# sbokov/AddingDisparityFiltering

Measured on AMD Instinct MI355X. Metric: filtered Mpixels/s (+ achieved HBM GB/s) on 4K disparity, 1/2/4/8 GPUs vs CPU ref, higher is better.
Workload: dtype f32

## Files before the change

addingdisparityfiltering_amd/csrc/conf_kernels.hip:

```cpp
#include "adf_internal.h"
#include <mutex>
#include <cstdlib>
#include <type_traits>
#include "prep_bodies.h"

#pragma clang fp contract(off)

namespace adf {

namespace {

using namespace tile;
#define ADF_ST(p, v) __builtin_nontemporal_store((v), (p))
constexpr int MAX_RADIUS = 40;

template <class Sum2>
__device__ __forceinline__ float disc_value(int s1, Sum2 sum2, double scale, float roll_off)
{
    const float mean = (float)((double)s1 * scale);
    const float sq = (float)(sum2() * scale);
    const float variance = sq - mean * mean;
    const float v = 1.0f - roll_off * variance;
    return v < 0.0f ? 0.0f : v;
}

__global__ void __launch_bounds__(NT) discontinuity_kernel(DiscArgs a)
{
    extern __shared__ __align__(16) unsigned char smem[];
    const int r = a.radius, k = 2 * r + 1;
    const int IH = TY + 2 * r, IW = TX + 2 * r;
    const int IWP = IW | 1;
    long long* h2 = reinterpret_cast<long long*>(smem);
    int* h1 = reinterpret_cast<int*>(h2 + (size_t)IH * TX);
    int16_t* in = reinterpret_cast<int16_t*>(h1 + (size_t)IH * TX);

    const int tid = threadIdx.x, tx = tid & (TX - 1), ty = tid / TX;
    const int x0 = blockIdx.x * TX, y0 = blockIdx.y * TY;
    const int view = a.only_view >= 0 ? a.only_view : (int)(blockIdx.z & 1);
    const size_t pz = a.only_view >= 0 ? blockIdx.z : (blockIdx.z >> 1);
    const char* base = reinterpret_cast<const char*>(a.disp[view]) + (ptrdiff_t)pz * a.pair_stride[view];
    const int rx = a.rx[view];

    for (int yy = ty; yy < IH; yy += NT / TX) {
        const int gy = reflect101(y0 + yy - r, a.rh);
        const int16_t* row = reinterpret_cast<const int16_t*>(base + (ptrdiff_t)(a.ry + gy) * a.stride[view]) + rx;
        for (int xx = tx; xx < IW; xx += TX)
            in[yy * IWP + xx] = row[reflect101(x0 + xx - r, a.rw)];
    }
    __syncthreads();

    for (int item = tid; item < IH * 8; item += NT) {
        const int yy = item >> 3, xs = (item & 7) * 8;
        const int16_t* p = in + yy * IWP + xs;
        int s1 = 0; long long s2 = 0;
        for (int q = 0; q < k; q++) { const int v = p[q]; s1 += v; s2 += (long long)(v * v); }
        int* o1 = h1 + yy * TX + xs; long long* o2 = h2 + yy * TX + xs;
        o1[0] = s1; o2[0] = s2;
#pragma unroll
        for (int i = 1; i < 8; i++) {
            const int va = p[i + k - 1], vb = p[i - 1];
            s1 += va - vb; s2 += (long long)(va * va - vb * vb);
            o1[i] = s1; o2[i] = s2;
        }
    }
    __syncthreads();

    {
        const int ys = ty * 8;
        const double scale = 1.0 / ((double)k * (double)k);
        int s1 = 0; long long s2 = 0;
        for (int q = 0; q < k; q++) { s1 += h1[(ys + q) * TX + tx]; s2 += h2[(ys + q) * TX + tx]; }
        float* dst = a.dst[view] + pz * a.frame;
        const int gx = x0 + tx;
#pragma unroll
        for (int i = 0; i < 8; i++) {
            if (i > 0) {
                s1 += h1[(ys + i + k - 1) * TX + tx] - h1[(ys + i - 1) * TX + tx];
                s2 += h2[(ys + i + k - 1) * TX + tx] - h2[(ys + i - 1) * TX + tx];
            }
            const int gy = y0 + ys + i;
            if (gy < a.rh && gx < a.rw) {
                dst[(size_t)(a.ry + gy) * a.W + rx + gx] = disc_value(s1, [=] { return (double)s2; }, scale, a.roll_off);
            }
        }
    }
}

constexpr int CONF_GROUP = 8;
constexpr int LRC_GROUP = 4;
#define DC_ROWS ((rows_total + (int)gridDim.y - 1) / (int)gridDim.y)

inline int row_blocks(int rows, int blocks_xz)
{
    int rpb = 128;
    while (rpb > 16 && ((rows + rpb - 1) / rpb) * blocks_xz < 2048) rpb >>= 1;
    return (rows + rpb - 1) / rpb;
}

__device__ __forceinline__ void lds_barrier()
{
    asm volatile("s_waitcnt lgkmcnt(0)\n\ts_barrier" ::: "memory");
}

struct WinSum {
    int s1, lo, hi;
    __device__ __forceinline__ void clear() { s1 = 0; lo = 0; hi = 0; }
    __device__ __forceinline__ void tap(const int2 v) { s1 += v.x; lo += v.y & 0xffff; hi += (int)((unsigned)v.y >> 16); }
    __device__ __forceinline__ void add(const WinSum& o) { s1 += o.s1; lo += o.lo; hi += o.hi; }
    __device__ __forceinline__ void sub(const WinSum& o) { s1 -= o.s1; lo -= o.lo; hi -= o.hi; }
    __device__ __forceinline__ double sum2() const { return (double)hi * 65536.0 + (double)lo; }
    __device__ static __forceinline__ int2 stage(int d) { return make_int2(d, __mul24(d, d)); }
};

template <int RT>
__global__ void __launch_bounds__(NT) discontinuity_col_kernel(DiscArgs a)
{
    constexpr int K = 2 * RT + 1;
    constexpr int OUTW = NT - 2 * RT;
    __shared__ int2 rowbuf[2][NT];
    const int tid = threadIdx.x;
    const int rows_total = a.rh;
    const int view = a.only_view >= 0 ? a.only_view : (int)(blockIdx.z & 1);
    const size_t pz = a.only_view >= 0 ? blockIdx.z : (blockIdx.z >> 1);
    const int x_out0 = blockIdx.x * OUTW, y_out0 = blockIdx.y * DC_ROWS;
    const char* base = reinterpret_cast<const char*>(a.disp[view]) + (ptrdiff_t)pz * a.pair_stride[view];
    const int rx = a.rx[view];
    const int gx_in = reflect101(x_out0 - RT + tid, a.rw);
    const int gx_out = x_out0 + tid - RT;
    const bool writer = tid >= RT && tid < NT - RT && gx_out < a.rw;
    float* dst = a.dst[view] + pz * a.frame + (size_t)a.ry * a.W + rx + gx_out;
    const int nrows = min(DC_ROWS, a.rh - y_out0) + 2 * RT;
    const double scale = 1.0 / ((double)K * (double)K);

    auto load = [&](int n) -> int {
        const int gy = reflect101(y_out0 - RT + n, a.rh);
        return reinterpret_cast<const int16_t*>(base + (ptrdiff_t)(a.ry + gy) * a.stride[view])[rx + gx_in];
    };

    constexpr int U = K * ((CONF_GROUP + K - 1) / K);
    WinSum ring[K], S;
    S.clear();
    int nxt[U];
#pragma unroll
    for (int s = 0; s < U; s++) nxt[s] = (s < nrows) ? load(s) : 0;
    for (int n0 = 0; n0 < nrows; n0 += U) {
        int cur[U];
#pragma unroll
        for (int s = 0; s < U; s++) { cur[s] = nxt[s]; asm volatile("" : "+v"(cur[s])); }
#pragma unroll
        for (int s = 0; s < U; s++) nxt[s] = (n0 + U + s < nrows) ? load(n0 + U + s) : 0;
#pragma unroll
        for (int s = 0; s < U; s++) {
            const int n = n0 + s;
            const int slot = s % K;
            if (n < nrows) {
                rowbuf[n & 1][tid] = WinSum::stage(cur[s]);
                lds_barrier();
                WinSum hsum;
                hsum.clear();
                if (tid >= RT && tid < NT - RT) {
#pragma unroll
                    for (int d = -RT; d <= RT; d++) hsum.tap(rowbuf[n & 1][tid + d]);
                }
                if (n >= K) S.sub(ring[slot]);
                ring[slot] = hsum;
                S.add(hsum);
                if (n >= 2 * RT && writer) {
                    const int oy = y_out0 + n - 2 * RT;
                    ADF_ST(&dst[(size_t)oy * a.W], disc_value(S.s1, [&] { return S.sum2(); }, scale, a.roll_off));
                }
            }
        }
    }
}

template <int RT, bool WRITE_U>
__global__ void __launch_bounds__(NT) conf_left_kernel(ConfLeftArgs a)
{
    constexpr int K = 2 * RT + 1;
    constexpr int OUTW = NT - 2 * RT;
    constexpr int U = K * ((LRC_GROUP + K - 1) / K);
    constexpr int CR = RT > 0 ? RT : 1;
    __shared__ int2 rowbuf[2][NT];
    const Geom& g = a.g;
    const int tid = threadIdx.x;
    const int rows_total = g.rh;
    const size_t pz = blockIdx.z;
    const int x_out0 = blockIdx.x * OUTW, y_out0 = blockIdx.y * DC_ROWS;
    const char* baseL = reinterpret_cast<const char*>(a.dL) + (ptrdiff_t)pz * a.psL;
    const char* baseR = reinterpret_cast<const char*>(a.dR) + (ptrdiff_t)pz * a.psR;
    const float* cR = a.cR + pz * g.frame;
    float* conf = a.conf + pz * g.cframe + g.cx0;
    const int gx_in = reflect101(x_out0 - RT + tid, g.rw);
    const int gx_out = x_out0 + tid - RT;
    const bool writer = tid >= RT && tid < NT - RT && gx_out < g.rw;
    const int j_abs = g.rx + gx_out;
    const int rows_out = min(DC_ROWS, g.rh - y_out0);
    const int nrows = rows_out + 2 * RT;
    const double scale = 1.0 / ((double)K * (double)K);
    const int right_end = a.rrx + g.rw;

    auto load = [&](int n) -> int {
        const int gy = reflect101(y_out0 - RT + n, g.rh);
        return reinterpret_cast<const int16_t*>(baseL + (ptrdiff_t)(g.ry + gy) * a.sL)[g.rx + gx_in];
    };

    WinSum ring[K], S;
    S.clear();
    int nxt[U], cur[U];
    int gd[U]; float gc[U];
    int cd[CR], cdr[CR]; float ccr[CR];
#pragma unroll
    for (int k = 0; k < CR; k++) { cd[k] = 0; cdr[k] = 0; ccr[k] = 0.0f; }
#pragma unroll
    for (int s = 0; s < U; s++) nxt[s] = (s < nrows) ? load(s) : 0;
    for (int n0 = 0; n0 < nrows; n0 += U) {
#pragma unroll
        for (int s = 0; s < U; s++) { cur[s] = nxt[s]; asm volatile("" : "+v"(cur[s])); }
#pragma unroll
        for (int s = 0; s < U; s++) {
            const int n = n0 + s;
            gd[s] = 0; gc[s] = 0.0f;
            if (writer && n >= RT && n < nrows - RT) {
                const int ridx = j_abs - (cur[s] >> 4);
                if (ridx >= a.rrx && ridx < right_end) {
                    const int i_abs = g.ry + y_out0 + n - RT;
                    gd[s] = reinterpret_cast<const int16_t*>(baseR + (ptrdiff_t)i_abs * a.sR)[ridx];
                    gc[s] = cR[(size_t)i_abs * g.W + ridx];
                }
            }
        }
#pragma unroll
        for (int s = 0; s < U; s++) asm volatile("" : "+v"(gd[s]), "+v"(gc[s]));
#pragma unroll
        for (int s = 0; s < U; s++) nxt[s] = (n0 + U + s < nrows) ? load(n0 + U + s) : 0;
#pragma unroll
        for (int s = 0; s < U; s++) {
            const int n = n0 + s;
            const int slot = s % K;
            if (n < nrows) {
                rowbuf[n & 1][tid] = WinSum::stage(cur[s]);
                lds_barrier();
                WinSum hsum;
                hsum.clear();
                if (tid >= RT && tid < NT - RT) {
#pragma unroll
                    for (int d = -RT; d <= RT; d++) hsum.tap(rowbuf[n & 1][tid + d]);
                }
                if (n >= K) S.sub(ring[slot]);
                ring[slot] = hsum;
                S.add(hsum);
                if (n >= 2 * RT && writer) {
                    const int oy = y_out0 + n - 2 * RT;
                    const int i_abs = g.ry + oy;
                    float c = disc_value(S.s1, [&] { return S.sum2(); }, scale, a.roll_off);
                    const int d = (s >= RT) ? cur[(s >= RT) ? s - RT : 0] : cd[(s < RT) ? s : 0];
                    const int dr = (s >= RT) ? gd[(s >= RT) ? s - RT : 0] : cdr[(s < RT) ? s : 0];
                    const float b = (s >= RT) ? gc[(s >= RT) ? s - RT : 0] : ccr[(s < RT) ? s : 0];
                    const int ridx = j_abs - (d >> 4);
                    if (ridx >= a.rrx && ridx < right_end) {
                        if (abs(d + dr) < a.thresh) c = b < c ? b : c;
                        else c = 0.0f;
                    }
                    c = 255.0f * c;
                    ADF_ST(&conf[(size_t)i_abs * g.cpitch + j_abs], c);
                    if (WRITE_U) {
                        const RhsPlanes u = rhs_planes(a.U0, a.U1, ORIENT_PAIR, pz, g.plane);
                        const size_t o = rhs_index(ORIENT_PAIR, oy, gx_out, g);
                        u.U0[o] = c * (float)d;
                        u.U1[o] = c;
                    }
                }
            }
        }
#pragma unroll
        for (int k = 0; k < RT; k++) { cd[k] = cur[U - RT + k]; cdr[k] = gd[U - RT + k]; ccr[k] = gc[U - RT + k]; }
    }
}

constexpr int CB_COLS = 4;
#define CB_HALO(RT) (((RT) + CB_COLS - 1) / CB_COLS)
#define CB_WOUT(RT) ((64 - 2 * CB_HALO(RT)) * CB_COLS)
enum BandRing { RING_REGS, RING_LDS, RING_LDS_BY_WIDTH };
constexpr BandRing band_ring(int rt) { return rt < 4 ? RING_REGS : rt <= 6 ? RING_LDS : RING_LDS_BY_WIDTH; }
constexpr int CB_MAX_WAVES = 16;
constexpr int CB_MAX_BAND_ROWS = 2048;
constexpr int CB_MAX_RADIUS = 2 * CB_COLS;

__device__ __forceinline__ int dpp_from_prev(int v) { return __builtin_amdgcn_update_dpp(0, v, 0x138, 0xf, 0xf, false); }
__device__ __forceinline__ int dpp_from_next(int v) { return __builtin_amdgcn_update_dpp(0, v, 0x130, 0xf, 0xf, false); }

struct ColSum {
    int s1; unsigned lo; int hi;
    __device__ __forceinline__ void slide(int dn, int dold)
    {
        const int qn = __mul24(dn, dn), qo = __mul24(dold, dold);
        s1 += dn - dold;
        const int diff = qn - qo;
        lo += (unsigned)diff & 0xffffu;
        hi += diff >> 16;
    }
};

template <int J> __device__ __forceinline__ int dpp_prev_n(int v) { if constexpr (J <= 0) return v; else return dpp_prev_n<J - 1>(dpp_from_prev(v)); }
template <int J> __device__ __forceinline__ int dpp_next_n(int v) { if constexpr (J <= 0) return v; else return dpp_next_n<J - 1>(dpp_from_next(v)); }

template <int RT, int J>
__device__ __forceinline__ void band_neighbours(const int (&p1)[CB_COLS + 1], const unsigned (&pl)[CB_COLS + 1], const int (&ph)[CB_COLS + 1],
                                                int q, int& h1, unsigned& hl, int& hh)
{
    if constexpr (J >= 1) {
        const int mp = 4 - 4 * J + RT - q, mn = q + RT - 4 * J + 1;
        const int m = mp < 0 ? 0 : (mp > CB_COLS ? CB_COLS : mp), m2 = mn < 0 ? 0 : (mn > CB_COLS ? CB_COLS : mn);
        if (m > 0) {
            h1 += dpp_prev_n<J>(p1[CB_COLS] - p1[CB_COLS - m]); hl += (unsigned)dpp_prev_n<J>((int)(pl[CB_COLS] - pl[CB_COLS - m]));
            hh += dpp_prev_n<J>(ph[CB_COLS] - ph[CB_COLS - m]);
        }
        if (m2 > 0) { h1 += dpp_next_n<J>(p1[m2]); hl += (unsigned)dpp_next_n<J>((int)pl[m2]); hh += dpp_next_n<J>(ph[m2]); }
        band_neighbours<RT, J - 1>(p1, pl, ph, q, h1, hl, hh);
    }
}

template <int RT>
__device__ __forceinline__ void band_row_values(const ColSum (&V)[CB_COLS], double scale, float roll_off, float (&out)[CB_COLS])
{
    static_assert(RT >= 1 && RT <= 2 * CB_COLS, "the halo must fit two lanes");
    int p1[CB_COLS + 1], ph[CB_COLS + 1];
    unsigned pl[CB_COLS + 1];
    p1[0] = ph[0] = 0; pl[0] = 0u;
#pragma unroll
    for (int i = 0; i < CB_COLS; i++) { p1[i + 1] = p1[i] + V[i].s1; pl[i + 1] = pl[i] + V[i].lo; ph[i + 1] = ph[i] + V[i].hi; }
#pragma unroll
    for (int q = 0; q < CB_COLS; q++) {
        const int a = q - RT > 0 ? q - RT : 0, b = (q + RT < CB_COLS - 1 ? q + RT : CB_COLS - 1) + 1;
        int h1 = p1[b] - p1[a], hh = ph[b] - ph[a];
        unsigned hl = pl[b] - pl[a];
        band_neighbours<RT, CB_HALO(RT)>(p1, pl, ph, q, h1, hl, hh);
        out[q] = disc_value(h1, [=] { return __builtin_fma((double)hh, 65536.0, (double)hl); }, scale, roll_off);
    }
}

template <int RT, bool RLDS = band_ring(RT) != RING_REGS>
__device__ __forceinline__ void conf_band_body(const ConfBandArgs& a, const int band, const size_t pz, unsigned char* smem)
{
    constexpr int K = 2 * RT + 1;
    constexpr int RING = RLDS ? K + 1 : RT + 2;
    typedef int v2i_u __attribute__((ext_vector_type(2), aligned(2)));
    typedef float v4f_u __attribute__((ext_vector_type(4), aligned(4)));
    const Geom& g = a.g;
    const int rw = g.rw, rwp = (rw + 3) & ~3;
    float* crow = reinterpret_cast<float*>(smem);
    int16_t* draw = reinterpret_cast<int16_t*>(crow + 2 * rwp);
    const int tid = threadIdx.x, lane = tid & 63, wv = tid >> 6;
    const int y0 = band * a.rows_per_band;
    const int rows_out = min(a.rows_per_band, g.rh - y0);
    const int nrows = rows_out + 2 * RT;
    constexpr int HL = CB_HALO(RT);
    const int vbase = wv * CB_WOUT(RT) + CB_COLS * (lane - HL);
    const bool out_lane = lane >= HL && lane <= 63 - HL && vbase < rw;

    int lcol = vbase;
    unsigned perm0 = 0x03020100u, perm1 = 0x07060504u;
    if (!(vbase >= 0 && vbase + CB_COLS - 1 < rw)) {
        int rv[CB_COLS], lo_need = rw;
#pragma unroll
        for (int q = 0; q < CB_COLS; q++) {
            const int v = vbase + q;
            const int vc = v < -RT ? -RT : (v > rw - 1 + RT ? rw - 1 + RT : v);
            rv[q] = reflect101(vc, rw);
            if (v >= -RT && v <= rw - 1 + RT) lo_need = min(lo_need, rv[q]);
        }
        lcol = lo_need >= rw ? 0 : lo_need;
        lcol = max(0, min(lcol, rw - CB_COLS));
        unsigned sb[CB_COLS];
#pragma unroll
        for (int q = 0; q < CB_COLS; q++) {
            const unsigned e = (unsigned)max(0, min(rv[q] - lcol, CB_COLS - 1));
            sb[q] = (2u * e) | ((2u * e + 1u) << 8);
        }
        perm0 = sb[0] | (sb[1] << 16);
        perm1 = sb[2] | (sb[3] << 16);
    }
    const char* baseL = reinterpret_cast<const char*>(a.dL) + (ptrdiff_t)pz * a.psL + (ptrdiff_t)g.ry * a.sL + (ptrdiff_t)g.rx * 2;
    const char* baseR = reinterpret_cast<const char*>(a.dR) + (ptrdiff_t)pz * a.psR + (ptrdiff_t)g.ry * a.sR + (ptrdiff_t)a.rrx * 2;
    const unsigned lane_off = (unsigned)lcol * 2u;
    float* conf = a.conf + pz * g.cframe + (size_t)g.ry * g.cpitch + g.cx0 + g.rx;
    const double scale = 1.0 / ((double)K * (double)K);
    const int right_end = a.rrx + rw;

    auto load = [&](const char* base, ptrdiff_t stride, int n) -> v2i_u {
        const int nn = n < nrows ? n : nrows - 1;
        int gy = abs(y0 - RT + nn);
        gy = gy >= g.rh ? 2 * (g.rh - 1) - gy : gy;
        return *reinterpret_cast<const v2i_u*>(base + (ptrdiff_t)gy * stride + lane_off);
    };
    auto permute = [&](v2i_u p) -> int2 {
        return make_int2((int)__builtin_amdgcn_perm((unsigned)p.y, (unsigned)p.x, perm0),
                         (int)__builtin_amdgcn_perm((unsigned)p.y, (unsigned)p.x, perm1));
    };
#define CB_ELEM(P, q) ((q) == 0 ? (int)(short)((P).x & 0xffff) : (q) == 1 ? ((P).x >> 16) : (q) == 2 ? (int)(short)((P).y & 0xffff) : ((P).y >> 16))

    int2 ringL[K], ringR[RLDS ? 1 : K];
    ColSum VL[CB_COLS], VR[CB_COLS];
#pragma unroll
    for (int k = 0; k < K; k++) { ringL[k] = make_int2(0, 0); if (!RLDS) ringR[k] = make_int2(0, 0); }
    const bool unaligned_wave = RLDS && __builtin_amdgcn_ballot_w64((lcol & 3) != 0) != 0;
#pragma unroll
    for (int q = 0; q < CB_COLS; q++) { VL[q].s1 = VL[q].hi = 0; VL[q].lo = 0u; VR[q].s1 = VR[q].hi = 0; VR[q].lo = 0u; }

    v2i_u pfL0 = load(baseL, a.sL, 0), pfR0 = load(baseR, a.sR, 0);
    v2i_u pfL1 = load(baseL, a.sL, 1), pfR1 = load(baseR, a.sR, 1);
    for (int n0 = 0; n0 < nrows; n0 += K) {
#pragma unroll
        for (int s = 0; s < K; s++) {
            const int n = n0 + s;
            if (n < nrows) {
                const int2 curL = permute(pfL0), curR = permute(pfR0);
                pfL0 = pfL1; pfR0 = pfR1;
                pfL1 = load(baseL, a.sL, n + 2); pfR1 = load(baseR, a.sR, n + 2);
                int2 oldR;
                if constexpr (RLDS) {
                    const int16_t* rp = draw + (n >= K ? (n - K) % RING : 0) * rwp + lcol;
                    v2i_u q2;
                    if (unaligned_wave) q2 = *reinterpret_cast<const v2i_u*>(rp);
                    else { const int2 t = *reinterpret_cast<const int2*>(rp); q2.x = t.x; q2.y = t.y; }
                    oldR = permute(q2);
                    if (n < K) oldR = make_int2(0, 0);
                } else
                    oldR = ringR[s];
#pragma unroll
                for (int q = 0; q < CB_COLS; q++) {
                    VL[q].slide(CB_ELEM(curL, q), CB_ELEM(ringL[s], q));
                    VR[q].slide(CB_ELEM(curR, q), CB_ELEM(oldR, q));
                }
                ringL[s] = curL;
                if constexpr (!RLDS) ringR[s] = curR;
                float cl[CB_COLS], cr[CB_COLS];
                const bool complete = n >= 2 * RT;
                if (complete) {
                    band_row_values<RT>(VR, scale, a.roll_off, cr);
                    band_row_values<RT>(VL, scale, a.roll_off, cl);
                }
                if (out_lane) {
                    *reinterpret_cast<int2*>(draw + (n % RING) * rwp + vbase) = curR;
                    if (complete) *reinterpret_cast<float4*>(crow + (n & 1) * rwp + vbase) = make_float4(cr[0], cr[1], cr[2], cr[3]);
                }
                lds_barrier();
                if (complete && out_lane) {
                    const int oy = y0 + n - 2 * RT;
                    const int2 cen = ringL[(s + K - RT) % K];
                    const float* cb = crow + (n & 1) * rwp;
                    const int16_t* db = draw + ((n - RT) % RING) * rwp;
                    float res[CB_COLS];
#pragma unroll
                    for (int q = 0; q < CB_COLS; q++) {
                        const int d = CB_ELEM(cen, q);
                        const int ridx = g.rx + vbase + q - (d >> 4);
                        const bool hit = ridx >= a.rrx && ridx < right_end;
                        const int rr = hit ? ridx - a.rrx : 0;
                        const float b = cb[rr];
                        const int dr = db[rr];
                        const float cmin = b < cl[q] ? b : cl[q];
                        const float chit = abs(d + dr) < a.thresh ? cmin : 0.0f;
                        res[q] = 255.0f * (hit ? chit : cl[q]);
                    }
                    float* dst = conf + (size_t)oy * g.cpitch + vbase;
                    if (vbase + CB_COLS <= rw) {
                        const v4f_u o = {res[0], res[1], res[2], res[3]};
                        __builtin_nontemporal_store(o, reinterpret_cast<v4f_u*>(dst));
                    } else {
#pragma unroll
                        for (int q = 0; q < CB_COLS; q++)
                            if (vbase + q < rw) ADF_ST(&dst[q], res[q]);
                    }
                }
            }
        }
    }
#undef CB_ELEM
}

template <int RT, bool RLDS = band_ring(RT) != RING_REGS>
__global__ void __launch_bounds__(64 * CB_MAX_WAVES) conf_band_kernel(ConfBandArgs a)
{
    extern __shared__ __align__(16) unsigned char smem[];
    conf_band_body<RT, RLDS>(a, blockIdx.x, blockIdx.y, smem);
}

constexpr int OUT_ROWS = 16;

__device__ __forceinline__ void outside_body(const OutsideArgs& a, const int nAx, const int nA, const unsigned blk, const size_t pz)
{
    const Geom& g = a.g;
    char* out = a.out ? reinterpret_cast<char*>(a.out) + (ptrdiff_t)pz * a.pair_stride : nullptr;
    float* conf = a.conf ? a.conf + pz * g.cframe + g.cx0 : nullptr;
    if ((int)blk < nA) {
        const int bx = blk % nAx, by = blk / nAx;
        const int t = bx * NT + threadIdx.x;
        if (t >= g.W - g.rw) return;
        const int j = t < g.rx ? t : t + g.rw;
        const int i0 = g.ry + by * OUT_ROWS, i1 = min(i0 + OUT_ROWS, g.ry + g.rh);
        for (int i = i0; i < i1; i++) {
            if (out) store_fill(out, (ptrdiff_t)i * a.stride, j, a.fill, a.out_f32);
            if (conf) conf[(size_t)i * g.cpitch + j] = 0.0f;
        }
    } else {
        const size_t npix = (size_t)(g.H - g.rh) * g.W;
        size_t p = (size_t)(blk - nA) * (NT * OUT_ROWS) + threadIdx.x;
#pragma unroll 4
        for (int k = 0; k < OUT_ROWS; k++, p += NT) {
            if (p >= npix) break;
            int i = (int)(p / (size_t)g.W);
            const int j = (int)(p - (size_t)i * g.W);
            if (i >= g.ry) i += g.rh;
            if (out) store_fill(out, (ptrdiff_t)i * a.stride, j, a.fill, a.out_f32);
            if (conf) conf[(size_t)i * g.cpitch + j] = 0.0f;
        }
    }
}

__global__ void __launch_bounds__(NT) outside_kernel(OutsideArgs a, int nAx, int nA)
{
    outside_body(a, nAx, nA, blockIdx.x, blockIdx.z);
}

struct OutsideGrid { int nAx, nA; size_t nB; bool in_range; };
inline OutsideGrid outside_grid(const Geom& g)
{
    const int side = g.W - g.rw;
    const int nAx = (side + NT - 1) / NT, nA = side > 0 ? nAx * ((g.rh + OUT_ROWS - 1) / OUT_ROWS) : 0;
    const size_t nB = ((size_t)(g.H - g.rh) * g.W + (size_t)NT * OUT_ROWS - 1) / ((size_t)NT * OUT_ROWS);
    return OutsideGrid{nAx > 0 ? nAx : 1, nA, nB, nA + nB <= 0x7fffffffu};
}

struct PrepArgs {
    ConfBandArgs c; WeightArgs w; OutsideArgs o;
    int nC, nW, nWx, nWy, nOAx, nOA;
};

template <int CH, int RT>
__global__ void __launch_bounds__(64 * CB_MAX_WAVES) prep_small_kernel(PrepArgs a)
{
    extern __shared__ __align__(16) unsigned char smem[];
    __shared__ prep::WsShared<CH> ws;
    const unsigned b = blockIdx.x;
    const size_t pz = blockIdx.y;
    if ((int)b < a.nC) {
        conf_band_body<RT>(a.c, (int)b, pz, smem);
    } else if ((int)b < a.nC + a.nW) {
        const int k = (int)b - a.nC;
        prep::weights_stream_body<CH>(a.w, k % a.nWx, k / a.nWx, a.nWy, pz, ws, threadIdx.x < prep::WS_NT);
    } else {
        if (threadIdx.x < NT) outside_body(a.o, a.nOAx, a.nOA, b - (unsigned)(a.nC + a.nW), pz);
    }
}

inline size_t disc_lds_bytes(int r)
{
    const size_t IH = TY + 2 * r, IWP = (TX + 2 * r) | 1;
    return IH * TX * 8 + IH * TX * 4 + ((IH * IWP * 2 + 15) & ~(size_t)15);
}

template <int LO, int HI, class F>
inline auto dispatch_radius(int radius, F&& f) -> decltype(f(std::integral_constant<int, LO>{}))
{
    if (radius == LO) return f(std::integral_constant<int, LO>{});
    if constexpr (LO < HI) return dispatch_radius<LO + 1, HI>(radius, f);
    else return nullptr;
}

template <class Kernel>
inline hipError_t ensure_dynamic_lds(Kernel kernel, size_t bytes, size_t threshold)
{
    if (bytes <= threshold) return hipSuccess;
    return hipFuncSetAttribute(reinterpret_cast<const void*>(kernel), hipFuncAttributeMaxDynamicSharedMemorySize, (int)bytes);
}

inline dim3 col_grid(int rw, int rh, int radius, int nz)
{
    const int gx = (rw + (NT - 2 * radius) - 1) / (NT - 2 * radius);
    return dim3(gx, row_blocks(rh, gx * nz), nz);
}

}

int max_disc_radius() { return MAX_RADIUS; }

hipError_t launch_discontinuity(const DiscArgs& a, int n_pairs, hipStream_t st)
{
    if (a.rw <= 0 || a.rh <= 0 || n_pairs <= 0) return hipSuccess;
    if (a.radius < 0 || a.radius > MAX_RADIUS) return hipErrorInvalidValue;
    const int nz = (a.only_view >= 0 ? 1 : 2) * n_pairs;
    if (a.radius <= 8) {
        const auto k = dispatch_radius<0, 8>(a.radius, [](auto R) { return &discontinuity_col_kernel<decltype(R)::value>; });
        hipLaunchKernelGGL(k, col_grid(a.rw, a.rh, a.radius, nz), dim3(NT), 0, st, a);
        return hipGetLastError();
    }
    static_assert(TX == 64 && TY == 32 && NT == 256, "discontinuity_kernel assumes a 64x32 tile and 256 threads");
    const size_t lds = disc_lds_bytes(a.radius);
    hipError_t e = ensure_dynamic_lds(discontinuity_kernel, lds, 48 * 1024);
    if (e != hipSuccess) return e;
    dim3 grid((a.rw + TX - 1) / TX, (a.rh + TY - 1) / TY, nz);
    hipLaunchKernelGGL(discontinuity_kernel, grid, dim3(NT), lds, st, a);
    return hipGetLastError();
}

int conf_left_max_radius() { return 8; }

constexpr size_t CB_LDS_LIMIT = 150 * 1024;

struct BandShape { int waves; size_t lds; bool rlds; };
static BandShape conf_band_shape(const Geom& g, int radius)
{
    const size_t rwp = (size_t)((g.rw + 3) & ~3);
    const auto lds = [&](size_t ring_rows) { return 2 * rwp * 4 + ring_rows * rwp * 2; };
    const size_t K = 2 * (size_t)radius + 1;
    const bool rlds = band_ring(radius) != RING_REGS && lds(K + 1) <= CB_LDS_LIMIT;
    return BandShape{(g.rw + CB_WOUT(radius) - 1) / CB_WOUT(radius), lds(rlds ? K + 1 : (size_t)radius + 2), rlds};
}

bool conf_band_fits(const Geom& g, int radius)
{
    return radius >= 1 && radius <= CB_MAX_RADIUS && g.rw >= 8 && g.rw > radius && g.rw <= CB_MAX_WAVES * CB_WOUT(radius) &&
           g.rh > radius && conf_band_shape(g, radius).lds <= CB_LDS_LIMIT;
}

typedef void (*BandKernel)(ConfBandArgs);
static BandKernel conf_band_variant(int radius, bool rlds)
{
    return dispatch_radius<1, CB_MAX_RADIUS>(radius, [&](auto R) -> BandKernel {
        constexpr int RR = decltype(R)::value;
        if constexpr (band_ring(RR) == RING_LDS_BY_WIDTH) return rlds ? conf_band_kernel<RR, true> : conf_band_kernel<RR, false>;
        else return conf_band_kernel<RR>;
    });
}

static int conf_band_resident(int radius, const BandShape& sh, int dev)
{
    struct Memo { int dev; BandShape sh; int value; };
    static Memo memo[CB_MAX_RADIUS + 1] = {};
    static std::mutex mu;
    {
        std::lock_guard<std::mutex> lk(mu);
        const Memo& m = memo[radius];
        if (m.value > 0 && m.dev == dev && m.sh.waves == sh.waves && m.sh.lds == sh.lds && m.sh.rlds == sh.rlds) return m.value;
    }
    int v = 0;
    const hipError_t e = hipOccupancyMaxActiveBlocksPerMultiprocessor(&v, conf_band_variant(radius, sh.rlds), 64 * sh.waves, sh.lds);
    if (e != hipSuccess || v < 1) { (void)hipGetLastError(); v = 1; }
    std::lock_guard<std::mutex> lk(mu);
    memo[radius] = Memo{dev, sh, v};
    return v;
}

static int cu_count(int dev)
{
    static int cache[64] = {0};
    int cus = 0;
    if (dev >= 0 && dev < 64) cus = __atomic_load_n(&cache[dev], __ATOMIC_RELAXED);
    if (cus <= 0) {
        if (dev < 0 || hipDeviceGetAttribute(&cus, hipDeviceAttributeMultiprocessorCount, dev) != hipSuccess || cus <= 0) cus = 256;
        if (dev >= 0 && dev < 64) __atomic_store_n(&cache[dev], cus, __ATOMIC_RELAXED);
    }
    return cus;
}

static int conf_band_clamp_rows(int want, int rh, int radius)
{
    const int min_rpb = 2 * radius > 4 ? 2 * radius : 4;
    int rpb = want < min_rpb ? min_rpb : want;
    if (rpb > CB_MAX_BAND_ROWS) rpb = CB_MAX_BAND_ROWS;
    return rpb > rh ? rh : rpb;
}

static int conf_band_rows_per_band(const Geom& g, int radius, const BandShape& sh, int n_pairs)
{
    static const int bands_env = [] { const char* e = getenv("ADF_CONF_BANDS_TOTAL"); return e ? atoi(e) : 0; }();
    int bands_total = bands_env;
    if (bands_total <= 0) {
        int dev = 0;
        if (hipGetDevice(&dev) != hipSuccess) dev = -1;
        const int cus = cu_count(dev);
        const int per_cu = conf_band_resident(radius, sh, dev);
        const int quarters = radius <= 5 && per_cu == 1 ? 4 : 3;
        bands_total = cus * quarters / 4 * per_cu;
    }
    const int bands = (bands_total + n_pairs - 1) / n_pairs;
    return conf_band_clamp_rows((g.rh + bands - 1) / bands, g.rh, radius);
}

hipError_t launch_conf_band(const ConfBandArgs& a0, int n_pairs, hipStream_t st)
{
    if (!conf_band_fits(a0.g, a0.radius)) return hipErrorInvalidValue;
    ConfBandArgs a = a0;
    const BandShape sh = conf_band_shape(a.g, a.radius);
    a.rows_per_band = conf_band_rows_per_band(a.g, a.radius, sh, n_pairs);
    const dim3 grid((a.g.rh + a.rows_per_band - 1) / a.rows_per_band, n_pairs), block(64 * sh.waves);
    const BandKernel k = conf_band_variant(a.radius, sh.rlds);
    if (!k) return hipErrorInvalidValue;
    hipError_t e = ensure_dynamic_lds(k, sh.lds, 48 * 1024);
    if (e != hipSuccess) return e;
    hipLaunchKernelGGL(k, grid, block, sh.lds, st, a);
    return hipGetLastError();
}

bool prep_small_fits(const Geom& g, int radius, int channels, int n_pairs)
{
    return conf_band_fits(g, radius) && radius <= 5 && (channels == 1 || channels == 3) &&
           (double)g.rw * g.rh * n_pairs <= 2.5e6;
}

bool prep_small_guide_fits(const Geom& g, ptrdiff_t guide_stride, int channels)
{
    return guide_stride > 0 && (size_t)(g.rh + 1) * (size_t)guide_stride < ((size_t)1 << 30) && (size_t)g.W * channels < ((size_t)1 << 29);
}

hipError_t launch_prep_small(const ConfBandArgs& c0, const WeightArgs& w, const OutsideArgs& o, int n_pairs, hipStream_t st)
{
    if (!prep_small_fits(c0.g, c0.radius, w.ch, n_pairs)) return hipErrorInvalidValue;
    if (!(w.chor_orient == ORIENT_N && w.cvert_orient == ORIENT_STRIP)) return hipErrorInvalidValue;
    if (!prep_small_guide_fits(c0.g, w.stride, w.ch)) return hipErrorInvalidValue;
    PrepArgs a{};
    a.c = c0; a.w = w; a.o = o;
    const Geom& g = c0.g;
    const BandShape sh = conf_band_shape(g, c0.radius);
    int waves = sh.waves;
    if (waves < prep::WS_NT / 64) waves = prep::WS_NT / 64;
    if (waves < NT / 64) waves = NT / 64;
    const int rows_all = g.rh * n_pairs;
    const int rpb = conf_band_clamp_rows((rows_all + 255) / 256, g.rh, c0.radius);
    a.c.rows_per_band = rpb;
    a.nC = (g.rh + rpb - 1) / rpb;
    a.nWx = (g.rw + prep::WS_BCOLS - 1) / prep::WS_BCOLS;
    int wrows = (rows_all * a.nWx + 511) / 512;
    if (wrows < 4) wrows = 4;
    a.nWy = (g.rh + wrows - 1) / wrows;
    a.nW = a.nWx * a.nWy;
    const OutsideGrid og = outside_grid(g);
    if (!og.in_range) return hipErrorInvalidValue;
    a.nOAx = og.nAx; a.nOA = og.nA;
    const dim3 grid(a.nC + a.nW + og.nA + (int)og.nB, n_pairs), block(64 * waves);
    if (sh.lds + sizeof(prep::WsShared<3>) > 150 * 1024) return hipErrorInvalidValue;
    const auto k = dispatch_radius<1, 5>(c0.radius, [&](auto R) {
        return w.ch == 1 ? &prep_small_kernel<1, decltype(R)::value> : &prep_small_kernel<3, decltype(R)::value>;
    });
    if (!k) return hipErrorInvalidValue;
    hipError_t e = ensure_dynamic_lds(k, sh.lds, 32 * 1024);
    if (e != hipSuccess) return e;
    hipLaunchKernelGGL(k, grid, block, sh.lds, st, a);
    return hipGetLastError();
}

hipError_t launch_conf_left(const ConfLeftArgs& a, int n_pairs, hipStream_t st)
{
    if (a.radius < 0 || a.radius > 8) return hipErrorInvalidValue;
    const auto k = dispatch_radius<0, 8>(a.radius, [&](auto R) {
        return a.U0 ? &conf_left_kernel<decltype(R)::value, true> : &conf_left_kernel<decltype(R)::value, false>;
    });
    hipLaunchKernelGGL(k, col_grid(a.g.rw, a.g.rh, a.radius, n_pairs), dim3(NT), 0, st, a);
    return hipGetLastError();
}

hipError_t launch_outside(const OutsideArgs& a, int n_pairs, hipStream_t st)
{
    const OutsideGrid og = outside_grid(a.g);
    if (og.nA + og.nB == 0) return hipSuccess;
    if (!og.in_range) return hipErrorInvalidValue;
    hipLaunchKernelGGL(outside_kernel, dim3((unsigned)(og.nA + og.nB), 1, n_pairs), dim3(NT), 0, st, a, og.nAx, og.nA);
    return hipGetLastError();
}

}
```

Baseline: 41250.

## Pack right-view confidence and disparity into LDS slots and simplify band lookup

For the register-ring path, the band kernel now writes each right-view confidence together with its biased centre disparity into a single interleaved LDS slot, so the lookup does one 8-byte read instead of two separate reads. The hit test and threshold check become unsigned range comparisons on precomputed bias and span values, and the float min is done on the raw bits. The column-sum update computes the difference of squares as (dn-dold)(dn+dold), saving a multiply. DPP moves use bound_ctrl, and global loads are steered toward scalar base plus vector offset addressing. The register path's LDS footprint changes to the slot layout, and the RING constant is now always K+1.

Result: no change. 41410, median of 6 (+0.4%).

```diff
diff --git a/addingdisparityfiltering_amd/csrc/conf_kernels.hip b/addingdisparityfiltering_amd/csrc/conf_kernels.hip
--- a/addingdisparityfiltering_amd/csrc/conf_kernels.hip
+++ b/addingdisparityfiltering_amd/csrc/conf_kernels.hip
@@ -287,16 +287,16 @@
 constexpr int CB_MAX_BAND_ROWS = 2048;
 constexpr int CB_MAX_RADIUS = 2 * CB_COLS;
 
-__device__ __forceinline__ int dpp_from_prev(int v) { return __builtin_amdgcn_update_dpp(0, v, 0x138, 0xf, 0xf, false); }
-__device__ __forceinline__ int dpp_from_next(int v) { return __builtin_amdgcn_update_dpp(0, v, 0x130, 0xf, 0xf, false); }
+__device__ __forceinline__ int dpp_from_prev(int v) { return __builtin_amdgcn_update_dpp(0, v, 0x138, 0xf, 0xf, true); }
+__device__ __forceinline__ int dpp_from_next(int v) { return __builtin_amdgcn_update_dpp(0, v, 0x130, 0xf, 0xf, true); }
 
 struct ColSum {
     int s1; unsigned lo; int hi;
     __device__ __forceinline__ void slide(int dn, int dold)
     {
-        const int qn = __mul24(dn, dn), qo = __mul24(dold, dold);
-        s1 += dn - dold;
-        const int diff = qn - qo;
+        const int t = dn - dold;
+        s1 += t;
+        const int diff = __mul24(t, dn + dold);
         lo += (unsigned)diff & 0xffffu;
         hi += diff >> 16;
     }
@@ -344,13 +344,14 @@
 __device__ __forceinline__ void conf_band_body(const ConfBandArgs& a, const int band, const size_t pz, unsigned char* smem)
 {
     constexpr int K = 2 * RT + 1;
-    constexpr int RING = RLDS ? K + 1 : RT + 2;
+    constexpr int RING = K + 1;
     typedef int v2i_u __attribute__((ext_vector_type(2), aligned(2)));
     typedef float v4f_u __attribute__((ext_vector_type(4), aligned(4)));
     const Geom& g = a.g;
     const int rw = g.rw, rwp = (rw + 3) & ~3;
     float* crow = reinterpret_cast<float*>(smem);
     int16_t* draw = reinterpret_cast<int16_t*>(crow + 2 * rwp);
+    int2* slot = reinterpret_cast<int2*>(smem);
     const int tid = threadIdx.x, lane = tid & 63, wv = tid >> 6;
     const int y0 = band * a.rows_per_band;
     const int rows_out = min(a.rows_per_band, g.rh - y0);
@@ -386,13 +387,24 @@
     const unsigned lane_off = (unsigned)lcol * 2u;
     float* conf = a.conf + pz * g.cframe + (size_t)g.ry * g.cpitch + g.cx0 + g.rx;
     const double scale = 1.0 / ((double)K * (double)K);
-    const int right_end = a.rrx + rw;
+    const int near_t = a.thresh < 0 ? 0 : (a.thresh > 65537 ? 65537 : a.thresh);
+    const int near_bias = near_t - 1;
+    unsigned near_span = near_t > 0 ? 2u * (unsigned)near_t - 1u : 0u;
+    int look0 = g.rx + vbase - a.rrx;
+    near_span = __builtin_amdgcn_readfirstlane(near_span);
+    asm("" : "+v"(look0));
 
     auto load = [&](const char* base, ptrdiff_t stride, int n) -> v2i_u {
         const int nn = n < nrows ? n : nrows - 1;
         int gy = abs(y0 - RT + nn);
         gy = gy >= g.rh ? 2 * (g.rh - 1) - gy : gy;
-        return *reinterpret_cast<const v2i_u*>(base + (ptrdiff_t)gy * stride + lane_off);
+        unsigned long long rowp = reinterpret_cast<unsigned long long>(base + (ptrdiff_t)gy * stride);
+        asm("" : "+s"(rowp));
+        typedef const __attribute__((address_space(1))) char* gchar_p;
+        typedef const __attribute__((address_space(1))) v2i_u* gv2i_p;
+        unsigned off = lane_off;
+        asm("" : "+v"(off));
+        return *reinterpret_cast<gv2i_p>(reinterpret_cast<gchar_p>(rowp) + off);
     };
     auto permute = [&](v2i_u p) -> int2 {
         return make_int2((int)__builtin_amdgcn_perm((unsigned)p.y, (unsigned)p.x, perm0),
@@ -428,7 +440,7 @@
                     if (n < K) oldR = make_int2(0, 0);
                 } else
                     oldR = ringR[s];
-#pragma unroll
+    #pragma unroll
                 for (int q = 0; q < CB_COLS; q++) {
                     VL[q].slide(CB_ELEM(curL, q), CB_ELEM(ringL[s], q));
                     VR[q].slide(CB_ELEM(curR, q), CB_ELEM(oldR, q));
@@ -441,35 +453,47 @@
                     band_row_values<RT>(VR, scale, a.roll_off, cr);
                     band_row_values<RT>(VL, scale, a.roll_off, cl);
                 }
-                if (out_lane) {
-                    *reinterpret_cast<int2*>(draw + (n % RING) * rwp + vbase) = curR;
-                    if (complete) *reinterpret_cast<float4*>(crow + (n & 1) * rwp + vbase) = make_float4(cr[0], cr[1], cr[2], cr[3]);
+                if constexpr (RLDS) {
+                    if (out_lane) {
+                        *reinterpret_cast<int2*>(draw + (n % RING) * rwp + vbase) = curR;
+                        if (complete) *reinterpret_cast<float4*>(crow + (n & 1) * rwp + vbase) = make_float4(cr[0], cr[1], cr[2], cr[3]);
+                    }
+                } else if (complete && out_lane) {
+                    const int2 cenR = ringR[(s + K - RT) % K];
+                    int4* sp = reinterpret_cast<int4*>(slot + (n & 1) * rwp + vbase);
+                    sp[0] = make_int4(__float_as_int(cr[0]), CB_ELEM(cenR, 0) + near_bias, __float_as_int(cr[1]), CB_ELEM(cenR, 1) + near_bias);
+                    sp[1] = make_int4(__float_as_int(cr[2]), CB_ELEM(cenR, 2) + near_bias, __float_as_int(cr[3]), CB_ELEM(cenR, 3) + near_bias);
                 }
                 lds_barrier();
                 if (complete && out_lane) {
                     const int oy = y0 + n - 2 * RT;
                     const int2 cen = ringL[(s + K - RT) % K];
-                    const float* cb = crow + (n & 1) * rwp;
-                    const int16_t* db = draw + ((n - RT) % RING) * rwp;
                     float res[CB_COLS];
-#pragma unroll
+    #pragma unroll
                     for (int q = 0; q < CB_COLS; q++) {
                         const int d = CB_ELEM(cen, q);
-                        const int ridx = g.rx + vbase + q - (d >> 4);
-                        const bool hit = ridx >= a.rrx && ridx < right_end;
-                        const int rr = hit ? ridx - a.rrx : 0;
-                        const float b = cb[rr];
-                        const int dr = db[rr];
-                        const float cmin = b < cl[q] ? b : cl[q];
-                        const float chit = abs(d + dr) < a.thresh ? cmin : 0.0f;
-                        res[q] = 255.0f * (hit ? chit : cl[q]);
+                        const unsigned rr = (unsigned)(look0 + q - (d >> 4));
+                        const bool hit = rr < (unsigned)rw;
+                        const unsigned ri = min(rr, (unsigned)(rw - 1));
+                        unsigned b; int x;
+                        if constexpr (RLDS) {
+                            b = __float_as_uint(crow[(n & 1) * rwp + ri]);
+                            x = d + draw[((n - RT) % RING) * rwp + ri] + near_bias;
+                        } else {
+                            const int2 sl = slot[(n & 1) * rwp + ri];
+                            b = (unsigned)sl.x;
+                            x = d + sl.y;
+                        }
+                        const unsigned cmin = min(b, __float_as_uint(cl[q]));
+                        const unsigned chit = (unsigned)x < near_span ? cmin : 0u;
+                        res[q] = 255.0f * __uint_as_float(hit ? chit : __float_as_uint(cl[q]));
                     }
                     float* dst = conf + (size_t)oy * g.cpitch + vbase;
                     if (vbase + CB_COLS <= rw) {
                         const v4f_u o = {res[0], res[1], res[2], res[3]};
                         __builtin_nontemporal_store(o, reinterpret_cast<v4f_u*>(dst));
                     } else {
-#pragma unroll
+    #pragma unroll
                         for (int q = 0; q < CB_COLS; q++)
                             if (vbase + q < rw) ADF_ST(&dst[q], res[q]);
                     }
@@ -613,10 +637,10 @@
 static BandShape conf_band_shape(const Geom& g, int radius)
 {
     const size_t rwp = (size_t)((g.rw + 3) & ~3);
-    const auto lds = [&](size_t ring_rows) { return 2 * rwp * 4 + ring_rows * rwp * 2; };
     const size_t K = 2 * (size_t)radius + 1;
-    const bool rlds = band_ring(radius) != RING_REGS && lds(K + 1) <= CB_LDS_LIMIT;
-    return BandShape{(g.rw + CB_WOUT(radius) - 1) / CB_WOUT(radius), lds(rlds ? K + 1 : (size_t)radius + 2), rlds};
+    const size_t lds_ring = 2 * rwp * 4 + (K + 1) * rwp * 2, lds_slots = 2 * rwp * 8;
+    const bool rlds = band_ring(radius) != RING_REGS && lds_ring <= CB_LDS_LIMIT;
+    return BandShape{(g.rw + CB_WOUT(radius) - 1) / CB_WOUT(radius), rlds ? lds_ring : lds_slots, rlds};
 }
 
 bool conf_band_fits(const Geom& g, int radius)
```
